# microfossil/particle-object-detection

Hardware: NVIDIA B200
Metric: detections_per_sec_posthead_path (higher is better)
Workload: dtype f32

## Files before the change

miso_b200/csrc/api.cu:

```cuda
#include "common.cuh"

extern "C" int mb_abi_version(void) { return MB_ABI_VERSION; }

extern "C" const char* mb_build_info(void) {
    return "libmisob200 sm_100a cuda " __DATE__
           ";kernels="
           "k_box_convert,k_box_decode,k_box_iou,k_box_max,k_clip_boxes,k_crop_gather,k_crop_plan,"
           "k_crop_plan_chunks,k_det_candidates,k_det_finalize,k_det_init,k_emit_single,k_emit_sorted,"
           "k_grid_anchors,k_group_hist,k_image_transform,k_kept_bucket,k_mask_prob,k_match_best,k_match_finish,"
           "k_mosaic_pack,k_mosaic_unpack,k_nchw_to_nhwc,k_nms_fixpoint,k_nms_mask,k_nms_sweep,k_nms_sweep_small,"
           "k_nms_sweep_wide,k_paste_masks,k_rank_in_segment,k_remove_small,k_resize_boxes,k_roi_align_backward,"
           "k_roi_align_direct,k_roi_align_nhwc,k_roi_align_nhwc4d,k_roi_align_sr2,k_roi_align_staged,"
           "k_roi_align_tma,k_roi_geom,k_rpn_decode,k_rpn_finalize,k_rpn_hist,k_rpn_select,k_scatter_boxes,"
           "k_seam_emit,k_seam_finish,k_seam_pairs,k_seam_prep,k_seam_resolve,k_seam_select,k_seg_meta,"
           "k_single_segment";
}
```

miso_b200/csrc/detpost.cu:

```cuda
#include <math.h>

#include "boxmath.cuh"
#include "nms_core.cuh"
#include "sort_smem.cuh"

namespace mb {

constexpr int kDetThreads = 256;
constexpr int kDetFinalThreads = 1024;
constexpr int kDetSortCap = 16384;
constexpr int kDetMergeMaxRuns = 8;

struct DetDev {
    int N, C, max_props, dpi;
    float score_thresh, min_size;
    DecodeWeights dw;
};
struct DetImages {
    int h[MB_MAX_IMAGES], w[MB_MAX_IMAGES];
    float ratio_h[MB_MAX_IMAGES], ratio_w[MB_MAX_IMAGES];
};

struct DetScratch {
    float* img_max;
    unsigned long long* bkey;
    float4* bbox;
    int* bseg;
    unsigned long long* skey;
    float4* sbox;
    float4* box_by_flat;
    float* score_by_flat;
    float* seg_offset;
    unsigned long long* keepbits;
    unsigned long long* mask;
    unsigned long long* gkeys;
    int gcap;
    SegArrays seg;
    size_t zero_bytes;
    long long mask_words;
    long long P;
};

static void carve_det(Carver& c, DetScratch& w, const DetDev& d) {
    const int G = d.N * (d.C - 1);
    const long long P = (long long)G * d.max_props;
    w.P = P;
    w.img_max = c.take<float>(d.N);
    w.seg = carve_seg_arrays(c, G);
    w.zero_bytes = align_up(c.off, 16);
    w.bkey = c.take<unsigned long long>(P);
    w.bbox = c.take<float4>(P);
    w.bseg = c.take<int>(P);
    w.skey = c.take<unsigned long long>(P);
    w.sbox = c.take<float4>(P);
    w.box_by_flat = c.take<float4>(P);
    w.score_by_flat = c.take<float>(P);
    w.seg_offset = c.take<float>(G);
    w.keepbits = c.take<unsigned long long>((size_t)G * (d.max_props / 64 + 2));
    w.mask_words = (long long)G * d.max_props * ((d.max_props + 63) / 64);
    w.mask = c.take<unsigned long long>((size_t)w.mask_words);
    const long long per_seg = d.max_props < d.dpi ? d.max_props : d.dpi;
    const long long bound = (long long)(d.C - 1) * per_seg;
    w.gcap = bound > kDetSortCap ? next_pow2((int)bound) : 0;
    w.gkeys = w.gcap ? c.take<unsigned long long>((size_t)d.N * w.gcap) : nullptr;
}

__global__ void __launch_bounds__(kDetThreads) k_det_candidates(const DetDev d, const DetImages im,
                                                               const float* __restrict__ logits,
                                                               const float* __restrict__ reg,
                                                               const float4* __restrict__ proposals,
                                                               const int* __restrict__ prop_counts, int packed,
                                                               DetScratch w) {
    pdl_enter();
    const int t = blockIdx.x * kDetThreads + threadIdx.x;
    if (t >= d.N * d.max_props) return;
// ... 41 lines not shown
    for (long long j = i; j < zero_vecs; j += stride) {
        uint4 v = make_uint4(0u, 0u, 0u, 0u);
        const long long s = j - seg_start_vec;
        if (s >= 0 && s < seg_vecs) {
            const long long g0 = 4 * s;
            v.x = g0 < G ? (unsigned)(g0 * max_props) : 0u;
            v.y = g0 + 1 < G ? (unsigned)((g0 + 1) * max_props) : 0u;
            v.z = g0 + 2 < G ? (unsigned)((g0 + 2) * max_props) : 0u;
            v.w = g0 + 3 < G ? (unsigned)((g0 + 3) * max_props) : 0u;
        }
        zero16[j] = v;
    }
    for (long long j = i; j < P; j += stride) bseg[j] = -1;
}

__global__ void __launch_bounds__(kDetFinalThreads) k_det_finalize(const DetDev d, const DetImages im, DetScratch w,
                                                                  float4* det_boxes, float4* det_boxes_net,
                                                                  float* det_scores, long long* det_labels,
                                                                  int* det_counts, int use_merge, int smem_keys) {
    pdl_enter();
    extern __shared__ __align__(16) unsigned long long keys_smem[];
    unsigned long long* keys = keys_smem;
    __shared__ int s_cnt;
    __shared__ int run_off[kDetMergeMaxRuns + 1];
    __shared__ int wpre[kDetMergeMaxRuns][kSweepSmallMaxWords + 1];
    const int n = blockIdx.x, tid = threadIdx.x;
    const int S = d.C - 1, F = d.max_props * S;
    int total;
    if (use_merge) {
        for (int i = tid; i < S * (kSweepSmallMaxWords + 1); i += kDetFinalThreads) {
            const int c = i / (kSweepSmallMaxWords + 1), q = i - c * (kSweepSmallMaxWords + 1);
            const int g = n * S + c;
            wpre[c][q] = (q < w.seg.seg_words[g]) ? __popcll(w.keepbits[w.seg.keep_off[g] + q]) : 0;
        }
        __syncthreads();
        if (tid < S) {
            const int T = w.seg.seg_words[n * S + tid];
            int acc = 0;
            for (int q = 0; q < T; ++q) { const int cq = wpre[tid][q]; wpre[tid][q] = acc; acc += cq; }
            wpre[tid][T] = acc;
        }
        __syncthreads();
        if (tid == 0) {
            int acc = 0;
            for (int c = 0; c < S; ++c) { run_off[c] = acc; acc += wpre[c][w.seg.seg_words[n * S + c]]; }
            run_off[S] = acc;
        }
        __syncthreads();
        total = run_off[S];
        for (int c = 0; c < S; ++c) {
            const int g = n * S + c;
            const int cnt = w.seg.seg_count[g], st = w.seg.seg_start[g];
            const unsigned long long* kb = w.keepbits + w.seg.keep_off[g];
            for (int q = tid; q < cnt; q += kDetFinalThreads) {
                const unsigned long long word = kb[q >> 6];
                if ((word >> (q & 63)) & 1ull)
                    keys[total + run_off[c] + wpre[c][q >> 6] + __popcll(word & ((1ull << (q & 63)) - 1ull))] = w.skey[st + q];
            }
        }
        __syncthreads();
        for (int e = tid; e < total; e += kDetFinalThreads) {
            int c = 0;
            while (e >= run_off[c + 1]) ++c;
            const int rank = merged_rank(keys + total, run_off, S, c, e - run_off[c]);
            keys[rank] = keys[total + e];
        }
        __syncthreads();
    } else {
        if (tid == 0) s_cnt = 0;
        __syncthreads();
        if (w.gcap) {
            int local = 0;
            for (int c = 0; c < S; ++c) {
                const int g = n * S + c;
                const unsigned long long* kb = w.keepbits + w.seg.keep_off[g];
                for (int q = tid; q < w.seg.seg_words[g]; q += kDetFinalThreads) local += __popcll(kb[q]);
            }
            if (local) atomicAdd(&s_cnt, local);
            __syncthreads();
            if (next_pow2(max(s_cnt, 2)) > smem_keys) keys = w.gkeys + (size_t)n * w.gcap;
            __syncthreads();
            if (tid == 0) s_cnt = 0;
            __syncthreads();
        }
        for (int c = 0; c < S; ++c) {
            const int g = n * S + c;
            const int cnt = w.seg.seg_count[g], st = w.seg.seg_start[g];
            const unsigned long long* kb = w.keepbits + w.seg.keep_off[g];
            for (int q0 = 0; q0 < cnt; q0 += kDetFinalThreads) {
                const int q = q0 + tid;
                const bool kept = q < cnt && ((kb[q >> 6] >> (q & 63)) & 1ull);
                const int slot = warp_alloc_slot(&s_cnt, kept);
                if (kept) keys[slot] = w.skey[st + q];
            }
        }
        __syncthreads();
        total = s_cnt;
        const int np2 = next_pow2(max(total, 2));
        for (int i = total + tid; i < np2; i += kDetFinalThreads) keys[i] = ~0ull;
        bitonic_sort_smem(keys, np2);
    }
    const int nout = min(total, d.dpi);
    for (int i = tid; i < d.dpi; i += kDetFinalThreads) {
        float4 b = make_float4(0, 0, 0, 0);
        float s = 0.0f;
        long long lab = 0;
        if (i < nout) {
            const int flat = (int)(keys[i] & 0xffffffffull);
            b = w.box_by_flat[(size_t)n * F + flat];
            s = w.score_by_flat[(size_t)n * F + flat];
            lab = flat % S + 1;
        }
        const size_t o = (size_t)n * d.dpi + i;
        if (det_boxes_net != nullptr) det_boxes_net[o] = b;
        det_boxes[o] = (i < nout) ? resize_box(b, im.ratio_h[n], im.ratio_w[n]) : b;
        det_scores[o] = s;
        det_labels[o] = lab;
    }
    if (tid == 0) det_counts[n] = nout;
}

static int make_det(const mb_det_params& p, DetDev& d, DetImages& im) {
    if (p.num_images < 1 || p.num_images > MB_MAX_IMAGES || p.num_classes < 2 || p.max_props_per_image < 1 ||
        p.detections_per_img < 1)
        return MB_ERR_INVALID_ARG;
    d.N = p.num_images; d.C = p.num_classes; d.max_props = p.max_props_per_image; d.dpi = p.detections_per_img;
    d.score_thresh = p.score_thresh; d.min_size = p.min_size;
    d.dw = DecodeWeights{p.wx, p.wy, p.ww, p.wh, p.bbox_xform_clip};
    const long long per_seg = d.max_props < d.dpi ? d.max_props : d.dpi;
    if ((long long)(d.C - 1) * per_seg >= (1ll << 24)) return MB_ERR_UNSUPPORTED;
    if ((long long)d.N * (d.C - 1) * d.max_props >= (1ll << 30)) return MB_ERR_UNSUPPORTED;
    for (int n = 0; n < d.N; ++n) {
        im.h[n] = p.image_h[n]; im.w[n] = p.image_w[n];
        const bool rs = p.orig_h[n] > 0 && p.orig_w[n] > 0;
// ... 28 lines not shown
    DetDev d; DetImages im;
    int rc = make_det(*p, d, im);
    if (rc != MB_OK) return rc;
    Carver c(workspace, workspace_bytes);
    DetScratch w;
    carve_det(c, w, d);
    if (!c.ok()) return MB_ERR_WORKSPACE;
    const int G = d.N * (d.C - 1);
    if ((w.zero_bytes & 15) != 0 || (reinterpret_cast<uintptr_t>(workspace) & 15) != 0) return MB_ERR_INVALID_ARG;
    const size_t seg_start_off = (size_t)((const char*)w.seg.seg_start - (const char*)workspace);
    if ((seg_start_off & 15) != 0 || seg_start_off + 4 * (size_t)((G + 3) / 4 * 4) > w.zero_bytes) return MB_ERR_INVALID_ARG;
    MB_CUDA(launch_pdl(k_det_init, max(ceil_div(G, 256), 32), 256, 0, stream, G, d.max_props, (long long)(seg_start_off / 16),
                       (uint4*)workspace, (long long)(w.zero_bytes / 16), w.bseg, (long long)w.P));
    MB_CUDA(launch_pdl(k_det_candidates, ceil_div(d.N * d.max_props, kDetThreads), kDetThreads, 0, stream,
                       d, im, class_logits, box_regression, (const float4*)proposals, prop_counts, packed, w));
    MetaRule rule{d.C - 1, 1, p->trick_numel, w.img_max, w.seg_offset};
    MB_CUDA(launch_pdl(k_seg_meta, 1, 1024, 0, stream, w.seg, G, 0, w.mask_words, rule));
    MB_CUDA(launch_pdl(k_rank_in_segment, (int)ceil_div64(w.P, kRankKeys), kRankThreads, 0, stream,
                       w.bkey, w.bbox, w.bseg, w.seg.seg_start, w.seg.seg_count, nullptr, (int)w.P, w.skey, w.sbox));
    rc = launch_mask_and_sweep(w.sbox, w.seg, G, d.max_props, p->nms_thresh, w.mask, w.keepbits, d.dpi, stream, w.seg_offset);
    if (rc != MB_OK) return rc;
    const long long per_seg = d.max_props < d.dpi ? d.max_props : d.dpi;
    const int bound = (int)((d.C - 1) * per_seg);
    const int use_merge = (d.C - 1) <= kDetMergeMaxRuns && d.max_props <= 64 * kSweepSmallMaxWords && 2 * bound <= kDetSortCap;
    int cap = use_merge ? 2 * bound : next_pow2(bound > 2 ? bound : 2);
    if (cap > kDetSortCap) cap = kDetSortCap;
    const int smem = (cap > 2 ? cap : 2) * (int)sizeof(unsigned long long);
    MB_DYN_SMEM(k_det_finalize, smem);
    MB_CUDA(launch_pdl(k_det_finalize, d.N, kDetFinalThreads, smem, stream, d, im, w, (float4*)det_boxes, (float4*)det_boxes_net,
                       det_scores, (long long*)det_labels, det_counts, use_merge, cap));
    return MB_OK;
}
```

miso_b200/csrc/nms_core.cuh:

```cuda
#pragma once
#include <cstdlib>
#include "common.cuh"

namespace mb {

struct SegArrays {
    int* seg_start;
    int* seg_count;
    int* seg_words;
    long long* mask_off;
    long long* tile_pre;
    int* keep_off;
    int* seg_kept;
    long long* totals;
};

inline size_t seg_arrays_bytes(int G) {
    size_t b = 0;
    b += align_up(sizeof(int) * G, 256) * 4;
    b += align_up(sizeof(long long) * G, 256);
    b += align_up(sizeof(long long) * (G + 1), 256);
    b += align_up(sizeof(int) * (G + 1), 256);
    b += 256;
    return b + 256;
}

inline SegArrays carve_seg_arrays(Carver& c, int G) {
    SegArrays s;
    s.seg_start = c.take<int>(G);
    s.seg_count = c.take<int>(G);
    s.seg_words = c.take<int>(G);
    s.seg_kept = c.take<int>(G);
    s.mask_off = c.take<long long>(G);
    s.tile_pre = c.take<long long>(G + 1);
    s.keep_off = c.take<int>(G + 1);
    s.totals = c.take<long long>(4);
    return s;
}

__device__ inline long long block_excl_scan_1024(long long v, long long* sh , long long& total) {
    const int tid = threadIdx.x, lane = tid & 31, wid = tid >> 5;
    long long x = v;
#pragma unroll
    for (int o = 1; o < 32; o <<= 1) {
        long long y = __shfl_up_sync(0xffffffffu, x, o);
        if (lane >= o) x += y;
    }
    if (lane == 31) sh[wid] = x;
    __syncthreads();
    if (wid == 0) {
        long long w = sh[lane];
#pragma unroll
        for (int o = 1; o < 32; o <<= 1) {
            long long y = __shfl_up_sync(0xffffffffu, w, o);
// ... 4 lines not shown
    __syncthreads();
    long long warp_base = wid ? sh[32 + wid - 1] : 0;
    total = sh[32 + 31];
    long long r = warp_base + x - v;
    __syncthreads();
    return r;
}

struct MetaRule {
    int segs_per_image;
    int group_base;
    long long trick_numel;
    const float* img_max;
    float* seg_offset;
};

static __global__ void __launch_bounds__(1024) k_seg_meta(SegArrays s, int G, int compute_starts,
                                                   long long mask_cap_words, MetaRule rule) {
    pdl_enter();
    __shared__ long long sh[64];
    __shared__ long long carry[4];
    const int tid = threadIdx.x;
    if (G <= 32) {
        if (tid < 32) {
            const int n = tid < G ? s.seg_count[tid] : 0;
            const long long T = (n + 63) >> 6;
            long long v[4] = {(long long)n, (long long)n * T, T * (T + 1) / 2, T}, inc[4];
#pragma unroll
            for (int q = 0; q < 4; ++q) {
                inc[q] = v[q];
// ... 47 lines not shown
            s.seg_words[g] = (int)T;
            s.mask_off[g] = c1 + mo;
            s.tile_pre[g] = c2 + tp;
            s.keep_off[g] = (int)(c3 + ko);
        }
        __syncthreads();
    }
    if (tid == 0) {
        s.tile_pre[G] = carry[2];
        s.keep_off[G] = (int)carry[3];
        s.totals[0] = carry[2];
        s.totals[1] = carry[1];
        s.totals[2] = carry[1] > mask_cap_words ? 1 : 0;
    }
    }
    if (rule.segs_per_image > 0) {
        for (int g = tid; g < G; g += 1024) {
            const int img = g / rule.segs_per_image;
            long long cnt = 0;
            for (int q = 0; q < rule.segs_per_image; ++q) cnt += s.seg_count[img * rule.segs_per_image + q];
            float off = 0.0f;
            if (rule.trick_numel >= 0 && 4 * cnt <= rule.trick_numel) {
                const float grp = (float)(rule.group_base + g % rule.segs_per_image);
                off = __fmul_rn(grp, __fadd_rn(rule.img_max[img], 1.0f));
            }
            rule.seg_offset[g] = off;
        }
    }
}

constexpr int kRankThreads = 256;
constexpr int kRankSplit = 8;
constexpr int kRankKeys = kRankThreads / kRankSplit;
constexpr int kRankTile = 2048;

static __global__ void __launch_bounds__(kRankThreads) k_rank_in_segment(
    const unsigned long long* __restrict__ bkey, const float4* __restrict__ bbox,
    const int* __restrict__ bseg, const int* __restrict__ seg_start,
    const int* __restrict__ seg_count, const float* __restrict__ seg_offset, int P,
    unsigned long long* __restrict__ skey, float4* __restrict__ sbox) {
    pdl_enter();
    __shared__ unsigned long long tile[kRankTile];
    __shared__ int s_lo, s_hi;
// ... 50 lines not shown
    const float xx2 = (b.z < a.z) ? b.z : a.z;
    const float yy2 = (b.w < a.w) ? b.w : a.w;
    float w = __fsub_rn(xx2, xx1); w = (0.0f < w) ? w : 0.0f;
    float h = __fsub_rn(yy2, yy1); h = (0.0f < h) ? h : 0.0f;
    const float inter = __fmul_rn(w, h);
    const float ovr = __fdiv_rn(inter, __fsub_rn(__fadd_rn(area_a, area_b), inter));
    return ovr >= thr_up;
}

__device__ __forceinline__ float4 offset_box(float4 b, float o) {
    return make_float4(__fadd_rn(b.x, o), __fadd_rn(b.y, o), __fadd_rn(b.z, o), __fadd_rn(b.w, o));
}

static __global__ void __launch_bounds__(128) k_nms_mask(const float4* __restrict__ sbox, SegArrays s, int G,
                                                 float thr_up, unsigned long long* __restrict__ mask,
                                                 const float* __restrict__ seg_offset, int full) {
    pdl_enter();
    __shared__ float4 cbox[64];
    __shared__ float carea[64];
    constexpr int kMaskSegCache = 256;
    __shared__ long long s_pre[kMaskSegCache + 1];
    __shared__ long long s_moff[kMaskSegCache];
    __shared__ int s_cnt[kMaskSegCache], s_st[kMaskSegCache];
    __shared__ float s_off[kMaskSegCache];
    const int tid = threadIdx.x;
    if (s.totals[2] != 0) return;
    const long long total = s.totals[0];
    const bool cached = G <= kMaskSegCache;
    if (cached) {
        for (int i = tid; i <= G; i += blockDim.x) {
            s_pre[i] = s.tile_pre[i];
            if (i < G) {
                s_moff[i] = s.mask_off[i]; s_cnt[i] = s.seg_count[i]; s_st[i] = s.seg_start[i];
                s_off[i] = seg_offset != nullptr ? seg_offset[i] : 0.0f;
            }
        }
    }
    __syncthreads();
    for (long long t = blockIdx.x; t < total; t += gridDim.x) {
        int g = 0, r = 0, c = 0;
        if ((tid & 31) == 0) {
            int lo = 0, hi = G;
            while (hi - lo > 1) {
                const int mid = (lo + hi) >> 1;
                if ((cached ? s_pre[mid] : s.tile_pre[mid]) <= t) lo = mid; else hi = mid;
            }
            g = lo;
            const long long TT = ((cached ? s_cnt[g] : s.seg_count[g]) + 63) >> 6;
            const long long tl = t - (cached ? s_pre[g] : s.tile_pre[g]);
            long long rr;
            if (TT <= 2048) {
                const float d = (float)(2 * TT + 1);
                rr = (long long)((d - sqrtf(fmaxf(d * d - 8.0f * (float)tl, 0.0f))) * 0.5f);
            } else {
                const double d = (double)(2 * TT + 1);
                rr = (long long)((d - sqrt(d * d - 8.0 * (double)tl)) * 0.5);
            }
            if (rr < 0) rr = 0;
            if (rr > TT - 1) rr = TT - 1;
            while (rr + 1 <= TT - 1 && (rr + 1) * TT - (rr + 1) * rr / 2 <= tl) ++rr;
            while (rr > 0 && rr * TT - rr * (rr - 1) / 2 > tl) --rr;
            r = (int)rr; c = (int)(rr + (tl - (rr * TT - rr * (rr - 1) / 2)));
        }
        g = __shfl_sync(0xffffffffu, g, 0); r = __shfl_sync(0xffffffffu, r, 0); c = __shfl_sync(0xffffffffu, c, 0);
        const int n = cached ? s_cnt[g] : s.seg_count[g];
        const int st = cached ? s_st[g] : s.seg_start[g];
        const long long moff = cached ? s_moff[g] : s.mask_off[g];
        const float off = cached ? s_off[g] : (seg_offset != nullptr ? seg_offset[g] : 0.0f);
        const int T = (n + 63) >> 6;
        const int ncol = min(64, n - c * 64);
        const int row = r * 64 + (tid & 63), half = tid >> 6;
        float4 a_raw = make_float4(0.f, 0.f, 0.f, 0.f);
        if (row < n) a_raw = sbox[st + row];
        if (tid < ncol) {
            const float4 b = offset_box(sbox[st + c * 64 + tid], off);
            cbox[tid] = b;
            carea[tid] = box_area_rn(b);
        }
        __syncthreads();
        unsigned int word = 0;
        if (row < n) {
            const float4 a = offset_box(a_raw, off);
            const float area_a = box_area_rn(a);
// ... 26 lines not shown
            for (int j = 0; j < 32; ++j) {
                const unsigned int b = __ballot_sync(0xffffffffu, (word >> j) & 1u);
                if (lane == j) tw = b;
            }
            const int trow = c * 64 + 32 * half + lane;
            if (trow < n) reinterpret_cast<unsigned int*>(mask)[2 * (moff + (long long)r * n + trow) + sub] = tw;
        }
        __syncthreads();
    }
}

constexpr int kSweepThreads = 256;
constexpr int kSweepBigThreads = 1024;

static __global__ void __launch_bounds__(kSweepBigThreads) k_nms_sweep(SegArrays s, const unsigned long long* __restrict__ mask,
                                                                     unsigned long long* __restrict__ keepbits, int max_keep) {
    extern __shared__ unsigned long long removed[];
    __shared__ unsigned long long diag[64];
    __shared__ unsigned long long s_keepw;
    const int g = blockIdx.x, tid = threadIdx.x, lane = tid & 31, warp = tid >> 5;
    constexpr int kWarps = kSweepBigThreads / 32;
    const int n = s.seg_count[g];
    const int T = s.seg_words[g];
    const bool overflow = s.totals[2] != 0;
    if (n == 0 || overflow) { if (tid == 0) s.seg_kept[g] = 0; return; }
    const unsigned long long* m = mask + s.mask_off[g];
    unsigned long long* kb = keepbits + s.keep_off[g];
    for (int w = tid; w < T; w += kSweepBigThreads) removed[w] = 0;
    int kept = 0;
    for (int b = 0; b < T; ++b) {
        const int nb = min(64, n - b * 64);
        if (tid < 64) diag[tid] = tid < nb ? m[(long long)(b * 64 + tid) * T + b] : 0ull;
        __syncthreads();
        if (warp == 0) {
            const unsigned long long invalid = nb < 64 ? ~((1ull << nb) - 1ull) : 0ull;
            unsigned long long R = removed[b] | invalid, C = 0;
            const int t0 = lane, t1 = lane + 32;
            const unsigned long long s0 = diag[t0] & ((1ull << t0) - 1ull);
            const unsigned long long s1 = diag[t1] & ((1ull << t1) - 1ull);
            while ((C | R) != ~0ull) {
                const unsigned long long D = C | R;
                bool c0 = false, r0 = false, c1 = false, r1 = false;
// ... 24 lines not shown
            for (int c0 = b + 1 + lane; c0 < T; c0 += 32 * 8) {
                unsigned long long v[8];
#pragma unroll
                for (int u = 0; u < 8; ++u) { const int c = c0 + 32 * u; v[u] = c < T ? __ldg(row + c) : 0ull; }
#pragma unroll
                for (int u = 0; u < 8; ++u) if (v[u]) atomicOr(&removed[c0 + 32 * u], v[u]);
            }
        }
    }
    if (tid == 0) s.seg_kept[g] = kept;
}

constexpr int kSweepSmallMaxWords = 64;

static __global__ void __launch_bounds__(kSweepThreads) k_nms_sweep_small(SegArrays s, const unsigned long long* __restrict__ mask,
                                                                        unsigned long long* __restrict__ keepbits, int max_keep) {
    __shared__ unsigned long long removed[kSweepSmallMaxWords];
    __shared__ unsigned long long tile[64 * kSweepSmallMaxWords];
    __shared__ unsigned long long s_keepw;
    constexpr int kPre = 64 * kSweepSmallMaxWords / kSweepThreads;
    const int g = blockIdx.x, tid = threadIdx.x, lane = tid & 31, warp = tid >> 5;
    const int n = s.seg_count[g];
    const int T = s.seg_words[g];
    if (n == 0 || s.totals[2] != 0) { if (tid == 0) s.seg_kept[g] = 0; return; }
    const unsigned long long* m = mask + s.mask_off[g];
    unsigned long long* kb = keepbits + s.keep_off[g];
    if (tid < T) removed[tid] = 0;
    unsigned long long pre[kPre];
    static_assert(kPre == 16 && kSweepThreads == 256 && kSweepSmallMaxWords == 64, "prefetch mapping");
    auto prefetch = [&](int b) {
        const int nb = min(64, n - b * 64), Wn = T - b;
#pragma unroll
        for (int u = 0; u < kPre; ++u) {
            const int row = warp + 8 * (u >> 1), col = lane + 32 * (u & 1);
            pre[u] = (row < nb && col < Wn) ? m[(long long)(b * 64 + row) * T + b + col] : 0ull;
        }
    };
    prefetch(0);
    int kept = 0;
    for (int b = 0; b < T; ++b) {
        const int nb = min(64, n - b * 64), Wn = T - b;
// ... 38 lines not shown
                unsigned long long acc = 0, bits = (keepw >> (16 * q)) & 0xffffull;
                while (bits) {
                    const int t = __ffsll((long long)bits) - 1 + 16 * q; bits &= bits - 1;
                    acc |= tile[t * Wn + col];
                }
                if (acc) atomicOr(&removed[b + col], acc);
            }
        }
        __syncthreads();
    }
    if (tid == 0) s.seg_kept[g] = kept;
}

static __global__ void __launch_bounds__(kSweepThreads) k_nms_sweep_wide(SegArrays s, const unsigned long long* __restrict__ mask,
                                                                       unsigned long long* __restrict__ keepbits, int max_keep,
                                                                       int Tcap, int nbuf) {
    extern __shared__ unsigned long long wsm[];
    __shared__ unsigned long long s_keepw;
    unsigned long long* removed = wsm;
    unsigned long long* tiles = wsm + Tcap;
    const int g = blockIdx.x, tid = threadIdx.x, lane = tid & 31, warp = tid >> 5;
    const int n = s.seg_count[g];
    const int T = s.seg_words[g];
    if (n == 0 || s.totals[2] != 0) { if (tid == 0) s.seg_kept[g] = 0; return; }
    const unsigned long long* m = mask + s.mask_off[g];
    unsigned long long* kb = keepbits + s.keep_off[g];
    for (int w = tid; w < T; w += kSweepThreads) removed[w] = 0;
    auto stage = [&](int b, unsigned long long* dst) {
        const int nb = min(64, n - b * 64), Wn = T - b;
        for (int row = warp; row < nb; row += kSweepThreads / 32) {
            const unsigned long long* src = m + (long long)(b * 64 + row) * T + b;
            unsigned long long* d = dst + row * Wn;
            for (int col = lane; col < Wn; col += 32) {
                const unsigned da = (unsigned)__cvta_generic_to_shared(d + col);
                asm volatile("cp.async.ca.shared.global [%0], [%1], 8;" :: "r"(da), "l"(src + col) : "memory");
            }
        }
        asm volatile("cp.async.commit_group;" ::: "memory");
    };
    const size_t tile_words = (size_t)64 * Tcap;
    for (int q = 0; q < nbuf - 1; ++q) {
// ... 54 lines not shown
            acc |= __shfl_xor_sync(0xffffffffu, acc, 1);
            acc |= __shfl_xor_sync(0xffffffffu, acc, 2);
            if (q == 0 && col < Wn && acc) removed[b + col] |= acc;
        }
        if (nbuf == 1) {
            __syncthreads();
            if (b + 1 < T) stage(b + 1, tiles);
        }
    }
    if (tid == 0) s.seg_kept[g] = kept;
}

constexpr int kFixThreads = 1024;
constexpr int kFixWords = kFixThreads / 64;

static __global__ void __launch_bounds__(kFixThreads) k_nms_fixpoint(SegArrays s, const unsigned long long* __restrict__ mask,
                                                                     unsigned long long* __restrict__ keepbits, int max_keep) {
    pdl_enter();
    __shared__ __align__(8) unsigned int C32[2 * kFixWords], R32[2 * kFixWords];
    const int g = blockIdx.x, t = threadIdx.x, lane = t & 31, warp = t >> 5;
    const int n = s.seg_count[g];
    const int T = s.seg_words[g];
    if (n == 0 || s.totals[2] != 0) { if (t == 0) s.seg_kept[g] = 0; return; }
    const unsigned long long* m = mask + s.mask_off[g] + t;
    unsigned long long* kb = keepbits + s.keep_off[g];
    const int nw = min((warp >> 1) + 1, T);
    unsigned long long S[kFixWords];
#pragma unroll
    for (int w = 0; w < kFixWords; ++w) S[w] = (w < nw && t < n) ? m[(long long)w * n] : 0ull;
#pragma unroll
    for (int w = 0; w < kFixWords; ++w)
        if (w == (t >> 6)) S[w] &= (1ull << (t & 63)) - 1ull;
    bool decided = t >= n;
    {
        const unsigned int inv = __ballot_sync(0xffffffffu, decided);
        if (lane == 0) { C32[warp] = 0u; R32[warp] = inv; }
    }
    __syncthreads();
    const unsigned long long* Cw = reinterpret_cast<const unsigned long long*>(C32);
    const unsigned long long* Rw = reinterpret_cast<const unsigned long long*>(R32);
// ... 23 lines not shown
            unsigned long long keepw = Cw[b];
            if (max_keep > 0) {
                if (kept >= max_keep) keepw = 0ull;
                else if (kept + __popcll(keepw) > max_keep) {
                    int extra = kept + __popcll(keepw) - max_keep;
                    while (extra-- > 0) keepw &= ~(1ull << (63 - __clzll(keepw)));
                }
            }
            kb[b] = keepw;
            kept += __popcll(keepw);
        }
        s.seg_kept[g] = kept;
    }
}

inline bool sweep_in_order() {
    static const bool v = [] { const char* e = getenv("MB_NMS_SWEEP"); return e != nullptr && e[0] == 'b'; }();
    return v;
}

inline int sweep_smem_bytes(int max_words) { return max_words * (int)sizeof(unsigned long long); }

inline int launch_mask_and_sweep(const float4* sbox, SegArrays s, int G, int max_seg_elems, double iou_threshold,
                                 unsigned long long* mask, unsigned long long* keepbits, int max_keep,
                                 cudaStream_t stream, const float* seg_offset = nullptr) {
    const float thr_up = strict_gt_threshold(iou_threshold);
    const bool fix = max_seg_elems <= kFixThreads && !sweep_in_order();
    MB_CUDA(launch_pdl(k_nms_mask, num_sms() * 16, 128, 0, stream, sbox, s, G, thr_up, mask, seg_offset, fix ? 1 : 0));
    if (fix) {
        MB_CUDA(launch_pdl(k_nms_fixpoint, G, kFixThreads, 0, stream, s, mask, keepbits, max_keep));
        return MB_OK;
    }
    if (ceil_div(max_seg_elems, 64) <= kSweepSmallMaxWords) {
        k_nms_sweep_small<<<G, kSweepThreads, 0, stream>>>(s, mask, keepbits, max_keep);
        MB_LAUNCH_CHECK();
        return MB_OK;
    }
    {
        const int Tcap = ceil_div(max_seg_elems, 64);
        int nbuf = 4;
        while (nbuf > 1 && ((long long)Tcap + 64ll * nbuf * Tcap) * 8 > 200 * 1024) --nbuf;
        const long long bytes = ((long long)Tcap + 64ll * nbuf * Tcap) * 8;
        if (bytes <= 200 * 1024) {
            MB_DYN_SMEM(k_nms_sweep_wide, (int)bytes);
            k_nms_sweep_wide<<<G, kSweepThreads, (int)bytes, stream>>>(s, mask, keepbits, max_keep, Tcap, nbuf);
            MB_LAUNCH_CHECK();
            return MB_OK;
        }
    }
    const int smem = sweep_smem_bytes(ceil_div(max_seg_elems, 64) + 1);
    if (smem > 48 * 1024) {
        if (smem > 200 * 1024) return MB_ERR_UNSUPPORTED;
        MB_DYN_SMEM(k_nms_sweep, smem);
    }
    k_nms_sweep<<<G, kSweepBigThreads, smem, stream>>>(s, mask, keepbits, max_keep);
    MB_LAUNCH_CHECK();
    return MB_OK;
}

}
```

miso_b200/pipeline.py:

```python
from __future__ import annotations

import ctypes as C
import math
from dataclasses import dataclass
from typing import List, Sequence, Tuple

import torch
from torch import Tensor

from . import _lib
from ._lib import CropParams, DetParams, MisoB200Error, RoiAlignParams, RpnParams
from .detection import DetConfig, RpnConfig
from .ops import _ptr, base_anchors, infer_scale, level_thresholds


@dataclass
class HotPathShapes:
    num_images: int
    padded_image_size: Tuple[int, int]
    image_sizes: Sequence[Tuple[int, int]]
    original_image_sizes: Sequence[Tuple[int, int]]
    rpn_grids: Sequence[Tuple[int, int]]
    feature_grids: Sequence[Tuple[int, int]]
    channels: int = 256
    num_classes: int = 3
    pooled: int = 7
    sampling_ratio: int = 2
    image_channels: int = 3


class HotPath:
    KERNELS = {"mb_rpn_proposals": 7,
               "mb_multiscale_roi_align": 2,
               "mb_det_postprocess": 7,
               "mb_crop_plan": 1, "mb_crop_gather": 1}

    def __init__(self, shapes: HotPathShapes, rpn: RpnConfig, det: DetConfig, threshold: float = 0.5,
                 crop_capacity_bytes: int = 64 << 20, exact_roi_align: bool = True, device="cuda:0"):
        self.lib = _lib.load()
        self.s, self.dev = shapes, torch.device(device)
        n, R = shapes.num_images, int(rpn.post_nms_top_n)
        self.R, self.dpi = R, int(det.detections_per_img)
        dev = self.dev
        f32, i32, i64 = torch.float32, torch.int32, torch.int64
        self.proposals = torch.zeros((n, R, 4), dtype=f32, device=dev)
        self.prop_scores = torch.zeros((n, R), dtype=f32, device=dev)
        self.prop_counts = torch.zeros((n,), dtype=i32, device=dev)
        self.box_features = torch.empty((n * R, shapes.channels, shapes.pooled, shapes.pooled), dtype=f32, device=dev)
        self.det_boxes = torch.zeros((n, self.dpi, 4), dtype=f32, device=dev)
# ... 321 lines not shown
```

Before: 5.141 million.

## Fuse NMS fixpoint into det finalize and drop seg_meta via fixed segment layout

Segment offsets for mask, keepbits and starts are now computed from a fixed per-class capacity layout instead of a k_seg_meta prefix-scan kernel. The per-segment IoU offset is derived inline inside the mask kernel. The fixpoint NMS sweep is merged into the finalize kernel, with a per-image atomic ticket so the last class block of each image runs finalize. Together these cut the det-postprocess launch count from 7 to 5, at the cost of a larger fixed-capacity mask buffer, redundant per-segment count sums, and a threadfence/atomic handoff.

```diff
diff --git a/miso_b200/csrc/api.cu b/miso_b200/csrc/api.cu
--- a/miso_b200/csrc/api.cu
+++ b/miso_b200/csrc/api.cu
@@ -6,7 +6,7 @@
     return "libmisob200 sm_100a cuda " __DATE__
            ";kernels="
            "k_box_convert,k_box_decode,k_box_iou,k_box_max,k_clip_boxes,k_crop_gather,k_crop_plan,"
-           "k_crop_plan_chunks,k_det_candidates,k_det_finalize,k_det_init,k_emit_single,k_emit_sorted,"
+           "k_crop_plan_chunks,k_det_candidates,k_det_init,k_det_nms_finalize,k_emit_single,k_emit_sorted,"
            "k_grid_anchors,k_group_hist,k_image_transform,k_kept_bucket,k_mask_prob,k_match_best,k_match_finish,"
            "k_mosaic_pack,k_mosaic_unpack,k_nchw_to_nhwc,k_nms_fixpoint,k_nms_mask,k_nms_sweep,k_nms_sweep_small,"
            "k_nms_sweep_wide,k_paste_masks,k_rank_in_segment,k_remove_small,k_resize_boxes,k_roi_align_backward,"
diff --git a/miso_b200/csrc/detpost.cu b/miso_b200/csrc/detpost.cu
--- a/miso_b200/csrc/detpost.cu
+++ b/miso_b200/csrc/detpost.cu
@@ -30,14 +30,14 @@
     float4* sbox;
     float4* box_by_flat;
     float* score_by_flat;
-    float* seg_offset;
+    int* img_ticket;
     unsigned long long* keepbits;
     unsigned long long* mask;
     unsigned long long* gkeys;
     int gcap;
     SegArrays seg;
+    FixedSegs fx;
     size_t zero_bytes;
-    long long mask_words;
     long long P;
 };
 
@@ -45,7 +45,9 @@
     const int G = d.N * (d.C - 1);
     const long long P = (long long)G * d.max_props;
     w.P = P;
+    w.fx = fixed_segs(&d.max_props, 1, G);
     w.img_max = c.take<float>(d.N);
+    w.img_ticket = c.take<int>(d.N);
     w.seg = carve_seg_arrays(c, G);
     w.zero_bytes = align_up(c.off, 16);
     w.bkey = c.take<unsigned long long>(P);
@@ -55,10 +57,8 @@
     w.sbox = c.take<float4>(P);
     w.box_by_flat = c.take<float4>(P);
     w.score_by_flat = c.take<float>(P);
-    w.seg_offset = c.take<float>(G);
-    w.keepbits = c.take<unsigned long long>((size_t)G * (d.max_props / 64 + 2));
-    w.mask_words = (long long)G * d.max_props * ((d.max_props + 63) / 64);
-    w.mask = c.take<unsigned long long>((size_t)w.mask_words);
+    w.keepbits = c.take<unsigned long long>((size_t)w.fx.keep_words);
+    w.mask = c.take<unsigned long long>((size_t)w.fx.mask_words);
     const long long per_seg = d.max_props < d.dpi ? d.max_props : d.dpi;
     const long long bound = (long long)(d.C - 1) * per_seg;
     w.gcap = bound > kDetSortCap ? next_pow2((int)bound) : 0;
@@ -130,28 +130,26 @@
     for (long long j = i; j < P; j += stride) bseg[j] = -1;
 }
 
-__global__ void __launch_bounds__(kDetFinalThreads) k_det_finalize(const DetDev d, const DetImages im, DetScratch w,
-                                                                  float4* det_boxes, float4* det_boxes_net,
-                                                                  float* det_scores, long long* det_labels,
-                                                                  int* det_counts, int use_merge, int smem_keys) {
-    pdl_enter();
-    extern __shared__ __align__(16) unsigned long long keys_smem[];
-    unsigned long long* keys = keys_smem;
+__device__ void det_finalize_image(const DetDev& d, const DetImages& im, const DetScratch& w, int n,
+                                   unsigned long long* keys, float4* det_boxes, float4* det_boxes_net,
+                                   float* det_scores, long long* det_labels, int* det_counts, int use_merge,
+                                   int smem_keys) {
     __shared__ int s_cnt;
     __shared__ int run_off[kDetMergeMaxRuns + 1];
     __shared__ int wpre[kDetMergeMaxRuns][kSweepSmallMaxWords + 1];
-    const int n = blockIdx.x, tid = threadIdx.x;
+    const int tid = threadIdx.x;
     const int S = d.C - 1, F = d.max_props * S;
+    auto words = [&](int g) { return (w.seg.seg_count[g] + 63) >> 6; };
     int total;
     if (use_merge) {
         for (int i = tid; i < S * (kSweepSmallMaxWords + 1); i += kDetFinalThreads) {
             const int c = i / (kSweepSmallMaxWords + 1), q = i - c * (kSweepSmallMaxWords + 1);
             const int g = n * S + c;
-            wpre[c][q] = (q < w.seg.seg_words[g]) ? __popcll(w.keepbits[w.seg.keep_off[g] + q]) : 0;
+            wpre[c][q] = (q < words(g)) ? __popcll(__ldcg(&w.keepbits[fx_keep_off(w.fx, g) + q])) : 0;
         }
         __syncthreads();
         if (tid < S) {
-            const int T = w.seg.seg_words[n * S + tid];
+            const int T = words(n * S + tid);
             int acc = 0;
             for (int q = 0; q < T; ++q) { const int cq = wpre[tid][q]; wpre[tid][q] = acc; acc += cq; }
             wpre[tid][T] = acc;
@@ -159,17 +157,17 @@
         __syncthreads();
         if (tid == 0) {
             int acc = 0;
-            for (int c = 0; c < S; ++c) { run_off[c] = acc; acc += wpre[c][w.seg.seg_words[n * S + c]]; }
+            for (int c = 0; c < S; ++c) { run_off[c] = acc; acc += wpre[c][words(n * S + c)]; }
             run_off[S] = acc;
         }
         __syncthreads();
         total = run_off[S];
         for (int c = 0; c < S; ++c) {
             const int g = n * S + c;
-            const int cnt = w.seg.seg_count[g], st = w.seg.seg_start[g];
-            const unsigned long long* kb = w.keepbits + w.seg.keep_off[g];
+            const int cnt = w.seg.seg_count[g], st = fx_start(w.fx, g);
+            const unsigned long long* kb = w.keepbits + fx_keep_off(w.fx, g);
             for (int q = tid; q < cnt; q += kDetFinalThreads) {
-                const unsigned long long word = kb[q >> 6];
+                const unsigned long long word = __ldcg(&kb[q >> 6]);
                 if ((word >> (q & 63)) & 1ull)
                     keys[total + run_off[c] + wpre[c][q >> 6] + __popcll(word & ((1ull << (q & 63)) - 1ull))] = w.skey[st + q];
             }
@@ -189,8 +187,8 @@
             int local = 0;
             for (int c = 0; c < S; ++c) {
                 const int g = n * S + c;
-                const unsigned long long* kb = w.keepbits + w.seg.keep_off[g];
-                for (int q = tid; q < w.seg.seg_words[g]; q += kDetFinalThreads) local += __popcll(kb[q]);
+                const unsigned long long* kb = w.keepbits + fx_keep_off(w.fx, g);
+                for (int q = tid; q < words(g); q += kDetFinalThreads) local += __popcll(__ldcg(&kb[q]));
             }
             if (local) atomicAdd(&s_cnt, local);
             __syncthreads();
@@ -201,11 +199,11 @@
         }
         for (int c = 0; c < S; ++c) {
             const int g = n * S + c;
-            const int cnt = w.seg.seg_count[g], st = w.seg.seg_start[g];
-            const unsigned long long* kb = w.keepbits + w.seg.keep_off[g];
+            const int cnt = w.seg.seg_count[g], st = fx_start(w.fx, g);
+            const unsigned long long* kb = w.keepbits + fx_keep_off(w.fx, g);
             for (int q0 = 0; q0 < cnt; q0 += kDetFinalThreads) {
                 const int q = q0 + tid;
-                const bool kept = q < cnt && ((kb[q >> 6] >> (q & 63)) & 1ull);
+                const bool kept = q < cnt && ((__ldcg(&kb[q >> 6]) >> (q & 63)) & 1ull);
                 const int slot = warp_alloc_slot(&s_cnt, kept);
                 if (kept) keys[slot] = w.skey[st + q];
             }
@@ -234,6 +232,29 @@
         det_labels[o] = lab;
     }
     if (tid == 0) det_counts[n] = nout;
+}
+
+__global__ void __launch_bounds__(kDetFinalThreads) k_det_nms_finalize(const DetDev d, const DetImages im, DetScratch w,
+                                                                      int fixpoint, float4* det_boxes, float4* det_boxes_net,
+                                                                      float* det_scores, long long* det_labels,
+                                                                      int* det_counts, int use_merge, int smem_keys) {
+    pdl_enter();
+    extern __shared__ __align__(16) unsigned long long keys_smem[];
+    __shared__ int s_last;
+    int n = blockIdx.x;
+    if (fixpoint) {
+        const int g = blockIdx.x;
+        n = g / (d.C - 1);
+        nms_fixpoint_segment(w.seg, w.fx, g, w.mask, w.keepbits, d.dpi);
+        __threadfence();
+        __syncthreads();
+        if (threadIdx.x == 0) s_last = atomicAdd(&w.img_ticket[n], 1) == d.C - 2;
+        __syncthreads();
+        if (!s_last) return;
+        __threadfence();
+    }
+    det_finalize_image(d, im, w, n, keys_smem, det_boxes, det_boxes_net, det_scores, det_labels, det_counts, use_merge,
+                       smem_keys);
 }
 
 static int make_det(const mb_det_params& p, DetDev& d, DetImages& im) {
@@ -292,11 +313,12 @@
                        (uint4*)workspace, (long long)(w.zero_bytes / 16), w.bseg, (long long)w.P));
     MB_CUDA(launch_pdl(k_det_candidates, ceil_div(d.N * d.max_props, kDetThreads), kDetThreads, 0, stream,
                        d, im, class_logits, box_regression, (const float4*)proposals, prop_counts, packed, w));
-    MetaRule rule{d.C - 1, 1, p->trick_numel, w.img_max, w.seg_offset};
-    MB_CUDA(launch_pdl(k_seg_meta, 1, 1024, 0, stream, w.seg, G, 0, w.mask_words, rule));
     MB_CUDA(launch_pdl(k_rank_in_segment, (int)ceil_div64(w.P, kRankKeys), kRankThreads, 0, stream,
                        w.bkey, w.bbox, w.bseg, w.seg.seg_start, w.seg.seg_count, nullptr, (int)w.P, w.skey, w.sbox));
-    rc = launch_mask_and_sweep(w.sbox, w.seg, G, d.max_props, p->nms_thresh, w.mask, w.keepbits, d.dpi, stream, w.seg_offset);
+    const MetaRule rule{d.C - 1, 1, p->trick_numel, w.img_max};
+    const bool fix = fixpoint_sweep(d.max_props);
+    rc = launch_mask_and_sweep(w.sbox, w.seg, G, d.max_props, p->nms_thresh, w.mask, w.keepbits, d.dpi, stream, nullptr,
+                               w.fx, rule, true);
     if (rc != MB_OK) return rc;
     const long long per_seg = d.max_props < d.dpi ? d.max_props : d.dpi;
     const int bound = (int)((d.C - 1) * per_seg);
@@ -304,8 +326,8 @@
     int cap = use_merge ? 2 * bound : next_pow2(bound > 2 ? bound : 2);
     if (cap > kDetSortCap) cap = kDetSortCap;
     const int smem = (cap > 2 ? cap : 2) * (int)sizeof(unsigned long long);
-    MB_DYN_SMEM(k_det_finalize, smem);
-    MB_CUDA(launch_pdl(k_det_finalize, d.N, kDetFinalThreads, smem, stream, d, im, w, (float4*)det_boxes, (float4*)det_boxes_net,
-                       det_scores, (long long*)det_labels, det_counts, use_merge, cap));
+    MB_DYN_SMEM(k_det_nms_finalize, smem);
+    MB_CUDA(launch_pdl(k_det_nms_finalize, fix ? G : d.N, kDetFinalThreads, smem, stream, d, im, w, fix ? 1 : 0, (float4*)det_boxes,
+                       (float4*)det_boxes_net, det_scores, (long long*)det_labels, det_counts, use_merge, cap));
     return MB_OK;
 }
diff --git a/miso_b200/csrc/nms_core.cuh b/miso_b200/csrc/nms_core.cuh
--- a/miso_b200/csrc/nms_core.cuh
+++ b/miso_b200/csrc/nms_core.cuh
@@ -38,6 +38,70 @@
     return s;
 }
 
+constexpr int kFixedMaxPeriod = MB_MAX_LEVELS;
+
+struct FixedSegs {
+    int period;
+    int start[kFixedMaxPeriod + 1];
+    long long moff[kFixedMaxPeriod + 1];
+    long long tpre[kFixedMaxPeriod + 1];
+    int koff[kFixedMaxPeriod + 1];
+    long long tiles;
+    long long mask_words;
+    int keep_words;
+};
+
+inline FixedSegs fixed_segs(const int* cap, int period, int G) {
+    FixedSegs f = {};
+    f.period = period;
+    for (int j = 0; j < period; ++j) {
+        const long long T = (cap[j] + 63) / 64;
+        f.start[j + 1] = f.start[j] + cap[j];
+        f.moff[j + 1] = f.moff[j] + (long long)cap[j] * T;
+        f.tpre[j + 1] = f.tpre[j] + T * (T + 1) / 2;
+        f.koff[j + 1] = f.koff[j] + (int)T;
+    }
+    const int reps = G / period;
+    f.tiles = reps * f.tpre[period];
+    f.mask_words = reps * f.moff[period];
+    f.keep_words = reps * f.koff[period];
+    return f;
+}
+
+__host__ __device__ __forceinline__ int fx_start(const FixedSegs& f, int g) {
+    const int q = g / f.period, j = g - q * f.period;
+    return q * f.start[f.period] + f.start[j];
+}
+__device__ __forceinline__ long long fx_mask_off(const FixedSegs& f, int g) {
+    const int q = g / f.period, j = g - q * f.period;
+    return q * f.moff[f.period] + f.moff[j];
+}
+__device__ __forceinline__ long long fx_tile_pre(const FixedSegs& f, int g) {
+    const int q = g / f.period, j = g - q * f.period;
+    return q * f.tpre[f.period] + f.tpre[j];
+}
+__device__ __forceinline__ int fx_keep_off(const FixedSegs& f, int g) {
+    const int q = g / f.period, j = g - q * f.period;
+    return q * f.koff[f.period] + f.koff[j];
+}
+__device__ __forceinline__ int fx_cap_words(const FixedSegs& f, int g) {
+    const int j = g % f.period;
+    return f.koff[j + 1] - f.koff[j];
+}
+
+struct SegView { int n, T, koff; long long moff; bool skip; };
+__device__ __forceinline__ SegView seg_view(const SegArrays& s, const FixedSegs& f, int g) {
+    SegView v;
+    v.n = s.seg_count[g];
+    v.T = (v.n + 63) >> 6;
+    if (f.period > 0) {
+        v.moff = fx_mask_off(f, g); v.koff = fx_keep_off(f, g); v.skip = v.n == 0;
+    } else {
+        v.moff = s.mask_off[g]; v.koff = s.keep_off[g]; v.skip = v.n == 0 || s.totals[2] != 0;
+    }
+    return v;
+}
+
 __device__ inline long long block_excl_scan_1024(long long v, long long* sh , long long& total) {
     const int tid = threadIdx.x, lane = tid & 31, wid = tid >> 5;
     long long x = v;
@@ -72,6 +136,16 @@
     const float* img_max;
     float* seg_offset;
 };
+
+__device__ inline float rule_offset(const MetaRule& rule, const int* seg_count, int g) {
+    if (rule.segs_per_image <= 0 || rule.trick_numel < 0) return 0.0f;
+    const int img = g / rule.segs_per_image;
+    long long cnt = 0;
+    for (int q = 0; q < rule.segs_per_image; ++q) cnt += seg_count[img * rule.segs_per_image + q];
+    if (4 * cnt > rule.trick_numel) return 0.0f;
+    const float grp = (float)(rule.group_base + g % rule.segs_per_image);
+    return __fmul_rn(grp, __fadd_rn(rule.img_max[img], 1.0f));
+}
 
 static __global__ void __launch_bounds__(1024) k_seg_meta(SegArrays s, int G, int compute_starts,
                                                    long long mask_cap_words, MetaRule rule) {
@@ -149,19 +223,8 @@
         s.totals[2] = carry[1] > mask_cap_words ? 1 : 0;
     }
     }
-    if (rule.segs_per_image > 0) {
-        for (int g = tid; g < G; g += 1024) {
-            const int img = g / rule.segs_per_image;
-            long long cnt = 0;
-            for (int q = 0; q < rule.segs_per_image; ++q) cnt += s.seg_count[img * rule.segs_per_image + q];
-            float off = 0.0f;
-            if (rule.trick_numel >= 0 && 4 * cnt <= rule.trick_numel) {
-                const float grp = (float)(rule.group_base + g % rule.segs_per_image);
-                off = __fmul_rn(grp, __fadd_rn(rule.img_max[img], 1.0f));
-            }
-            rule.seg_offset[g] = off;
-        }
-    }
+    if (rule.segs_per_image > 0)
+        for (int g = tid; g < G; g += 1024) rule.seg_offset[g] = rule_offset(rule, s.seg_count, g);
 }
 
 constexpr int kRankThreads = 256;
@@ -242,26 +305,35 @@
 
 static __global__ void __launch_bounds__(128) k_nms_mask(const float4* __restrict__ sbox, SegArrays s, int G,
                                                  float thr_up, unsigned long long* __restrict__ mask,
-                                                 const float* __restrict__ seg_offset, int full) {
+                                                 const float* __restrict__ seg_offset, int full, FixedSegs fx,
+                                                 MetaRule rule) {
     pdl_enter();
     __shared__ float4 cbox[64];
     __shared__ float carea[64];
     constexpr int kMaskSegCache = 256;
     __shared__ long long s_pre[kMaskSegCache + 1];
     __shared__ long long s_moff[kMaskSegCache];
-    __shared__ int s_cnt[kMaskSegCache], s_st[kMaskSegCache];
+    __shared__ int s_cnt[kMaskSegCache], s_st[kMaskSegCache], s_T[kMaskSegCache];
     __shared__ float s_off[kMaskSegCache];
     const int tid = threadIdx.x;
-    if (s.totals[2] != 0) return;
-    const long long total = s.totals[0];
+    const bool fixed = fx.period > 0;
+    if (!fixed && s.totals[2] != 0) return;
+    const long long total = fixed ? fx.tiles : s.totals[0];
     const bool cached = G <= kMaskSegCache;
+    auto seg_meta = [&](int i, long long& pre, long long& moff, int& cnt, int& st, int& T, float& off) {
+        cnt = s.seg_count[i];
+        if (fixed) {
+            pre = fx_tile_pre(fx, i); moff = fx_mask_off(fx, i); st = fx_start(fx, i); T = fx_cap_words(fx, i);
+            off = rule_offset(rule, s.seg_count, i);
+        } else {
+            pre = s.tile_pre[i]; moff = s.mask_off[i]; st = s.seg_start[i]; T = (cnt + 63) >> 6;
+            off = seg_offset != nullptr ? seg_offset[i] : 0.0f;
+        }
+    };
     if (cached) {
         for (int i = tid; i <= G; i += blockDim.x) {
-            s_pre[i] = s.tile_pre[i];
-            if (i < G) {
-                s_moff[i] = s.mask_off[i]; s_cnt[i] = s.seg_count[i]; s_st[i] = s.seg_start[i];
-                s_off[i] = seg_offset != nullptr ? seg_offset[i] : 0.0f;
-            }
+            if (i < G) seg_meta(i, s_pre[i], s_moff[i], s_cnt[i], s_st[i], s_T[i], s_off[i]);
+            else s_pre[G] = fixed ? fx_tile_pre(fx, G) : s.tile_pre[G];
         }
     }
     __syncthreads();
@@ -271,11 +343,11 @@
             int lo = 0, hi = G;
             while (hi - lo > 1) {
                 const int mid = (lo + hi) >> 1;
-                if ((cached ? s_pre[mid] : s.tile_pre[mid]) <= t) lo = mid; else hi = mid;
+                if ((cached ? s_pre[mid] : fixed ? fx_tile_pre(fx, mid) : s.tile_pre[mid]) <= t) lo = mid; else hi = mid;
             }
             g = lo;
-            const long long TT = ((cached ? s_cnt[g] : s.seg_count[g]) + 63) >> 6;
-            const long long tl = t - (cached ? s_pre[g] : s.tile_pre[g]);
+            const long long TT = cached ? s_T[g] : fixed ? fx_cap_words(fx, g) : (s.seg_count[g] + 63) >> 6;
+            const long long tl = t - (cached ? s_pre[g] : fixed ? fx_tile_pre(fx, g) : s.tile_pre[g]);
             long long rr;
             if (TT <= 2048) {
                 const float d = (float)(2 * TT + 1);
@@ -291,10 +363,12 @@
             r = (int)rr; c = (int)(rr + (tl - (rr * TT - rr * (rr - 1) / 2)));
         }
         g = __shfl_sync(0xffffffffu, g, 0); r = __shfl_sync(0xffffffffu, r, 0); c = __shfl_sync(0xffffffffu, c, 0);
-        const int n = cached ? s_cnt[g] : s.seg_count[g];
-        const int st = cached ? s_st[g] : s.seg_start[g];
-        const long long moff = cached ? s_moff[g] : s.mask_off[g];
-        const float off = cached ? s_off[g] : (seg_offset != nullptr ? seg_offset[g] : 0.0f);
+        int n, st, Tg;
+        long long moff, pre;
+        float off;
+        if (cached) { n = s_cnt[g]; st = s_st[g]; moff = s_moff[g]; off = s_off[g]; }
+        else seg_meta(g, pre, moff, n, st, Tg, off);
+        if (c * 64 >= n) continue;
         const int T = (n + 63) >> 6;
         const int ncol = min(64, n - c * 64);
         const int row = r * 64 + (tid & 63), half = tid >> 6;
@@ -351,18 +425,18 @@
 constexpr int kSweepBigThreads = 1024;
 
 static __global__ void __launch_bounds__(kSweepBigThreads) k_nms_sweep(SegArrays s, const unsigned long long* __restrict__ mask,
-                                                                     unsigned long long* __restrict__ keepbits, int max_keep) {
+                                                                     unsigned long long* __restrict__ keepbits, int max_keep,
+                                                                     FixedSegs fx) {
     extern __shared__ unsigned long long removed[];
     __shared__ unsigned long long diag[64];
     __shared__ unsigned long long s_keepw;
     const int g = blockIdx.x, tid = threadIdx.x, lane = tid & 31, warp = tid >> 5;
     constexpr int kWarps = kSweepBigThreads / 32;
-    const int n = s.seg_count[g];
-    const int T = s.seg_words[g];
-    const bool overflow = s.totals[2] != 0;
-    if (n == 0 || overflow) { if (tid == 0) s.seg_kept[g] = 0; return; }
-    const unsigned long long* m = mask + s.mask_off[g];
-    unsigned long long* kb = keepbits + s.keep_off[g];
+    const SegView v = seg_view(s, fx, g);
+    const int n = v.n, T = v.T;
+    if (v.skip) { if (tid == 0) s.seg_kept[g] = 0; return; }
+    const unsigned long long* m = mask + v.moff;
+    unsigned long long* kb = keepbits + v.koff;
     for (int w = tid; w < T; w += kSweepBigThreads) removed[w] = 0;
     int kept = 0;
     for (int b = 0; b < T; ++b) {
@@ -417,17 +491,18 @@
 constexpr int kSweepSmallMaxWords = 64;
 
 static __global__ void __launch_bounds__(kSweepThreads) k_nms_sweep_small(SegArrays s, const unsigned long long* __restrict__ mask,
-                                                                        unsigned long long* __restrict__ keepbits, int max_keep) {
+                                                                        unsigned long long* __restrict__ keepbits, int max_keep,
+                                                                        FixedSegs fx) {
     __shared__ unsigned long long removed[kSweepSmallMaxWords];
     __shared__ unsigned long long tile[64 * kSweepSmallMaxWords];
     __shared__ unsigned long long s_keepw;
     constexpr int kPre = 64 * kSweepSmallMaxWords / kSweepThreads;
     const int g = blockIdx.x, tid = threadIdx.x, lane = tid & 31, warp = tid >> 5;
-    const int n = s.seg_count[g];
-    const int T = s.seg_words[g];
-    if (n == 0 || s.totals[2] != 0) { if (tid == 0) s.seg_kept[g] = 0; return; }
-    const unsigned long long* m = mask + s.mask_off[g];
-    unsigned long long* kb = keepbits + s.keep_off[g];
+    const SegView v = seg_view(s, fx, g);
+    const int n = v.n, T = v.T;
+    if (v.skip) { if (tid == 0) s.seg_kept[g] = 0; return; }
+    const unsigned long long* m = mask + v.moff;
+    unsigned long long* kb = keepbits + v.koff;
     if (tid < T) removed[tid] = 0;
     unsigned long long pre[kPre];
     static_assert(kPre == 16 && kSweepThreads == 256 && kSweepSmallMaxWords == 64, "prefetch mapping");
@@ -496,17 +571,17 @@
 
 static __global__ void __launch_bounds__(kSweepThreads) k_nms_sweep_wide(SegArrays s, const unsigned long long* __restrict__ mask,
                                                                        unsigned long long* __restrict__ keepbits, int max_keep,
-                                                                       int Tcap, int nbuf) {
+                                                                       int Tcap, int nbuf, FixedSegs fx) {
     extern __shared__ unsigned long long wsm[];
     __shared__ unsigned long long s_keepw;
     unsigned long long* removed = wsm;
     unsigned long long* tiles = wsm + Tcap;
     const int g = blockIdx.x, tid = threadIdx.x, lane = tid & 31, warp = tid >> 5;
-    const int n = s.seg_count[g];
-    const int T = s.seg_words[g];
-    if (n == 0 || s.totals[2] != 0) { if (tid == 0) s.seg_kept[g] = 0; return; }
-    const unsigned long long* m = mask + s.mask_off[g];
-    unsigned long long* kb = keepbits + s.keep_off[g];
+    const SegView v = seg_view(s, fx, g);
+    const int n = v.n, T = v.T;
+    if (v.skip) { if (tid == 0) s.seg_kept[g] = 0; return; }
+    const unsigned long long* m = mask + v.moff;
+    unsigned long long* kb = keepbits + v.koff;
     for (int w = tid; w < T; w += kSweepThreads) removed[w] = 0;
     auto stage = [&](int b, unsigned long long* dst) {
         const int nb = min(64, n - b * 64), Wn = T - b;
@@ -591,16 +666,16 @@
 constexpr int kFixThreads = 1024;
 constexpr int kFixWords = kFixThreads / 64;
 
-static __global__ void __launch_bounds__(kFixThreads) k_nms_fixpoint(SegArrays s, const unsigned long long* __restrict__ mask,
-                                                                     unsigned long long* __restrict__ keepbits, int max_keep) {
-    pdl_enter();
+__device__ inline void nms_fixpoint_segment(const SegArrays& s, const FixedSegs& fx, int g,
+                                            const unsigned long long* __restrict__ mask,
+                                            unsigned long long* __restrict__ keepbits, int max_keep) {
     __shared__ __align__(8) unsigned int C32[2 * kFixWords], R32[2 * kFixWords];
-    const int g = blockIdx.x, t = threadIdx.x, lane = t & 31, warp = t >> 5;
-    const int n = s.seg_count[g];
-    const int T = s.seg_words[g];
-    if (n == 0 || s.totals[2] != 0) { if (t == 0) s.seg_kept[g] = 0; return; }
-    const unsigned long long* m = mask + s.mask_off[g] + t;
-    unsigned long long* kb = keepbits + s.keep_off[g];
+    const int t = threadIdx.x, lane = t & 31, warp = t >> 5;
+    const SegView v = seg_view(s, fx, g);
+    const int n = v.n, T = v.T;
+    if (v.skip) { if (t == 0) s.seg_kept[g] = 0; return; }
+    const unsigned long long* m = mask + v.moff + t;
+    unsigned long long* kb = keepbits + v.koff;
     const int nw = min((warp >> 1) + 1, T);
     unsigned long long S[kFixWords];
 #pragma unroll
@@ -654,25 +729,35 @@
     }
 }
 
+static __global__ void __launch_bounds__(kFixThreads) k_nms_fixpoint(SegArrays s, const unsigned long long* __restrict__ mask,
+                                                                     unsigned long long* __restrict__ keepbits, int max_keep,
+                                                                     FixedSegs fx) {
+    pdl_enter();
+    nms_fixpoint_segment(s, fx, blockIdx.x, mask, keepbits, max_keep);
+}
+
 inline bool sweep_in_order() {
     static const bool v = [] { const char* e = getenv("MB_NMS_SWEEP"); return e != nullptr && e[0] == 'b'; }();
     return v;
 }
 
+inline bool fixpoint_sweep(int max_seg_elems) { return max_seg_elems <= kFixThreads && !sweep_in_order(); }
+
 inline int sweep_smem_bytes(int max_words) { return max_words * (int)sizeof(unsigned long long); }
 
 inline int launch_mask_and_sweep(const float4* sbox, SegArrays s, int G, int max_seg_elems, double iou_threshold,
                                  unsigned long long* mask, unsigned long long* keepbits, int max_keep,
-                                 cudaStream_t stream, const float* seg_offset = nullptr) {
+                                 cudaStream_t stream, const float* seg_offset = nullptr, FixedSegs fx = FixedSegs{},
+                                 MetaRule rule = MetaRule{}, bool caller_fixpoint = false) {
     const float thr_up = strict_gt_threshold(iou_threshold);
-    const bool fix = max_seg_elems <= kFixThreads && !sweep_in_order();
-    MB_CUDA(launch_pdl(k_nms_mask, num_sms() * 16, 128, 0, stream, sbox, s, G, thr_up, mask, seg_offset, fix ? 1 : 0));
+    const bool fix = fixpoint_sweep(max_seg_elems);
+    MB_CUDA(launch_pdl(k_nms_mask, num_sms() * 16, 128, 0, stream, sbox, s, G, thr_up, mask, seg_offset, fix ? 1 : 0, fx, rule));
     if (fix) {
-        MB_CUDA(launch_pdl(k_nms_fixpoint, G, kFixThreads, 0, stream, s, mask, keepbits, max_keep));
+        if (!caller_fixpoint) MB_CUDA(launch_pdl(k_nms_fixpoint, G, kFixThreads, 0, stream, s, mask, keepbits, max_keep, fx));
         return MB_OK;
     }
     if (ceil_div(max_seg_elems, 64) <= kSweepSmallMaxWords) {
-        k_nms_sweep_small<<<G, kSweepThreads, 0, stream>>>(s, mask, keepbits, max_keep);
+        k_nms_sweep_small<<<G, kSweepThreads, 0, stream>>>(s, mask, keepbits, max_keep, fx);
         MB_LAUNCH_CHECK();
         return MB_OK;
     }
@@ -683,7 +768,7 @@
         const long long bytes = ((long long)Tcap + 64ll * nbuf * Tcap) * 8;
         if (bytes <= 200 * 1024) {
             MB_DYN_SMEM(k_nms_sweep_wide, (int)bytes);
-            k_nms_sweep_wide<<<G, kSweepThreads, (int)bytes, stream>>>(s, mask, keepbits, max_keep, Tcap, nbuf);
+            k_nms_sweep_wide<<<G, kSweepThreads, (int)bytes, stream>>>(s, mask, keepbits, max_keep, Tcap, nbuf, fx);
             MB_LAUNCH_CHECK();
             return MB_OK;
         }
@@ -693,7 +778,7 @@
         if (smem > 200 * 1024) return MB_ERR_UNSUPPORTED;
         MB_DYN_SMEM(k_nms_sweep, smem);
     }
-    k_nms_sweep<<<G, kSweepBigThreads, smem, stream>>>(s, mask, keepbits, max_keep);
+    k_nms_sweep<<<G, kSweepBigThreads, smem, stream>>>(s, mask, keepbits, max_keep, fx);
     MB_LAUNCH_CHECK();
     return MB_OK;
 }
diff --git a/miso_b200/pipeline.py b/miso_b200/pipeline.py
--- a/miso_b200/pipeline.py
+++ b/miso_b200/pipeline.py
@@ -32,7 +32,7 @@
 class HotPath:
     KERNELS = {"mb_rpn_proposals": 7,
                "mb_multiscale_roi_align": 2,
-               "mb_det_postprocess": 7,
+               "mb_det_postprocess": 5,
                "mb_crop_plan": 1, "mb_crop_gather": 1}
 
     def __init__(self, shapes: HotPathShapes, rpn: RpnConfig, det: DetConfig, threshold: float = 0.5,
```

Result: no change. 5.157 million (median of 6 runs) (+0.3%).
